# luizirber/sourmash-rust

Measured on AMD Instinct MI355X. Metric: k-mers hashed/sec (k=31, scaled=1000), higher is better.
Workload: dtype u64

## Files before the change

sourmash-rust_amd/csrc/device.cpp:

```cpp
#include "device.hpp"

#include <cstdlib>
#include <cstring>

namespace smh {

void throw_hip(hipError_t e, const char* what, const char* file, int line) {
  std::string m = std::string("HIP error ") + hipGetErrorName(e) + " (" + hipGetErrorString(e) +
                  ") in " + what + " at " + file + ":" + std::to_string(line);
  throw_internal(m);
}

namespace {
std::mutex g_pool_mu;
std::map<std::pair<int, size_t>, std::vector<void*>> g_pool;
size_t g_pool_bytes = 0;
size_t g_pool_limit = [] {
  if (const char* e = std::getenv("SOURMASH_AMD_POOL_MB")) return (size_t)std::strtoull(e, nullptr, 10) << 20;
  return (size_t)1 << 30;
}();

size_t size_class(size_t need) {
  if (need <= 4096) return 4096;
  const int lg = 63 - __builtin_clzll((unsigned long long)(need - 1));
// ... 63 lines not shown
}
size_t device_pool_bytes() {
  std::lock_guard<std::mutex> lock(g_pool_mu);
  return g_pool_bytes;
}

void DeviceBuffer::ensure(size_t need) {
  if (need <= bytes) return;
  const size_t want = need + need / 4 + 4096;
  release();
  ptr = device_pool_alloc(want, &bytes);
}
void DeviceBuffer::release() {
  if (ptr) device_pool_free(ptr, bytes, true);
  ptr = nullptr;
  bytes = 0;
}
void DeviceBuffer::release_after_sync() {
  if (ptr) device_pool_free(ptr, bytes, false);
  ptr = nullptr;
  bytes = 0;
}
DeviceBuffer::~DeviceBuffer() { release(); }

void PinnedBuffer::ensure(size_t need) {
  if (need <= bytes) return;
  size_t want = need + need / 4 + 4096;
  if (ptr) { HIP_CHECK(hipHostFree(ptr)); ptr = nullptr; bytes = 0; }
  HIP_CHECK(hipHostMalloc(&ptr, want, hipHostMallocDefault));
  bytes = want;
}
PinnedBuffer::~PinnedBuffer() { if (ptr) (void)hipHostFree(ptr); }

static int pick_device() {
  if (const char* e = std::getenv("SOURMASH_AMD_DEVICE")) return std::atoi(e);
  int cur = 0;
  if (hipGetDevice(&cur) == hipSuccess) return cur;
  return 0;
}

Device::Device() {
  int n = 0;
  hipError_t e = hipGetDeviceCount(&n);
  if (e != hipSuccess || n <= 0)
    throw_internal("no HIP device available: the sourmash MI355X library needs a GPU (" +
                   std::string(e == hipSuccess ? "device count is 0" : hipGetErrorString(e)) + ")");
  device_ = pick_device();
  if (device_ < 0 || device_ >= n) device_ = 0;
  HIP_CHECK(hipSetDevice(device_));
  hipDeviceProp_t p;
  HIP_CHECK(hipGetDeviceProperties(&p, device_));
  cus_ = p.multiProcessorCount > 0 ? p.multiProcessorCount : 256;
  HIP_CHECK(hipStreamCreateWithFlags(&stream_, hipStreamNonBlocking));
  HIP_CHECK(hipStreamCreateWithFlags(&copy_stream_, hipStreamNonBlocking));
  HIP_CHECK(hipEventCreateWithFlags(&fence_, hipEventDisableTiming));
  HIP_CHECK(hipEventCreateWithFlags(&ev_fork_, hipEventDisableTiming));
  HIP_CHECK(hipEventCreateWithFlags(&ev_join_, hipEventDisableTiming));
  HIP_CHECK(hipEventCreateWithFlags(&open_event_, hipEventDisableTiming));
}

void Device::leave_open(hipStream_t s) {
  std::lock_guard<std::recursive_mutex> lock(mu_);
  HIP_CHECK(hipEventRecord(open_event_, s));
  open_stream_ = s;
  open_ = true;
}

void Device::order_after_open(hipStream_t s) {
  std::lock_guard<std::recursive_mutex> lock(mu_);
  if (!open_) return;
  if (hipEventQuery(open_event_) == hipSuccess) { open_ = false; return; }
  if (s != open_stream_) HIP_CHECK(hipStreamWaitEvent(s, open_event_, 0));
}

hipStream_t Device::user_stream(void* given) {
  std::lock_guard<std::recursive_mutex> lock(mu_);
  if (given) { order_after_open((hipStream_t)given); return (hipStream_t)given; }
  HIP_CHECK(hipEventRecord(fence_, nullptr));
  HIP_CHECK(hipStreamWaitEvent(stream_, fence_, 0));
  order_after_open(stream_);
  return stream_;
}

Device& Device::get() {
  static Device* d = new Device();
  (void)hipSetDevice(d->device_);
  return *d;
}

bool Device::available() {
  try {
    (void)get();
    return true;
  } catch (const Error&) {
    return false;
  }
}

void Device::profile_enable(bool on) { profiling_ = on; }

void Device::prof_begin(hipStream_t s) {
  if (!profiling_) return;
  HIP_CHECK(hipEventCreate(&cur_start_));
  HIP_CHECK(hipEventRecord(cur_start_, s));
}

void Device::prof_end(const char* name, hipStream_t s) {
  if (!profiling_ || !cur_start_) return;
  hipEvent_t b;
  HIP_CHECK(hipEventCreate(&b));
  HIP_CHECK(hipEventRecord(b, s));
  pending_.push_back({name, cur_start_, b});
  cur_start_ = nullptr;
  if (pending_.size() > 4096) drain();
}

void Device::drain() {
  for (auto& p : pending_) {
    float ms = 0.f;
    if (hipEventSynchronize(p.b) == hipSuccess && hipEventElapsedTime(&ms, p.a, p.b) == hipSuccess) {
      auto& t = times_[p.name];
      t.ms += ms;
      t.launches += 1;
    }
    (void)hipEventDestroy(p.a);
    (void)hipEventDestroy(p.b);
  }
  pending_.clear();
}

void Device::count(const char* name) {
  std::lock_guard<std::recursive_mutex> lock(mu_);
  times_[name].launches += 1;
}

KernelTimes Device::prof_get(const std::string& name) {
  drain();
  auto it = times_.find(name);
  return it == times_.end() ? KernelTimes{} : it->second;
}

void Device::prof_reset() {
  drain();
  times_.clear();
}

}
```

sourmash-rust_amd/csrc/device.hpp:

```cpp
#pragma once
#include <hip/hip_runtime.h>

#include <cstddef>
#include <cstdint>
#include <map>
#include <mutex>
#include <string>
#include <vector>

#include "common.hpp"

namespace smh {

[[noreturn]] void throw_hip(hipError_t e, const char* what, const char* file, int line);

#define HIP_CHECK(expr)                                                  \
  do {                                                                   \
    hipError_t e_ = (expr);                                              \
    if (e_ != hipSuccess) ::smh::throw_hip(e_, #expr, __FILE__, __LINE__); \
  } while (0)

void* device_pool_alloc(size_t need, size_t* cap);
void device_pool_free(void* ptr, size_t cap, bool sync);
void device_pool_trim();
void device_pool_set_limit(size_t bytes);
size_t device_pool_bytes();

struct PoolBlock {
  void* ptr = nullptr;
  size_t cap = 0;
  bool synced = false;
  explicit PoolBlock(size_t bytes) { ptr = device_pool_alloc(bytes ? bytes : 1, &cap); }
  PoolBlock(const PoolBlock&) = delete; PoolBlock& operator=(const PoolBlock&) = delete;
  ~PoolBlock() { device_pool_free(ptr, cap, !synced); }
  template <class T> T* as() const { return reinterpret_cast<T*>(ptr); }
};

struct DeviceBuffer {
  void* ptr = nullptr;
  size_t bytes = 0;
  void ensure(size_t need);
  void release();
  void release_after_sync();
  template <class T> T* as() const { return reinterpret_cast<T*>(ptr); }
  DeviceBuffer() = default;
  DeviceBuffer(const DeviceBuffer&) = delete;
  DeviceBuffer& operator=(const DeviceBuffer&) = delete;
  ~DeviceBuffer();
};

struct PinnedBuffer {
  void* ptr = nullptr;
  size_t bytes = 0;
  void ensure(size_t need);
  template <class T> T* as() const { return reinterpret_cast<T*>(ptr); }
  PinnedBuffer() = default;
  PinnedBuffer(const PinnedBuffer&) = delete;
  PinnedBuffer& operator=(const PinnedBuffer&) = delete;
  ~PinnedBuffer();
};

struct KernelTimes {
  double ms = 0.0;
  uint64_t launches = 0;
};

class Device {
 public:
  static Device& get();
  static bool available();

  int id() const { return device_; }
  int cu_count() const { return cus_; }
  hipStream_t stream() { order_after_open(stream_); return stream_; }
  hipStream_t copy_stream() const { return copy_stream_; }
  hipEvent_t fork_event() const { return ev_fork_; }
  hipEvent_t join_event() const { return ev_join_; }
  void leave_open(hipStream_t s);
  void order_after_open(hipStream_t s);
  hipStream_t user_stream(void* given);
  std::recursive_mutex& mutex() { return mu_; }

  DeviceBuffer scratch;
  DeviceBuffer tile_rec;

  void profile_enable(bool on);
  bool profiling() const { return profiling_; }
  void prof_begin(hipStream_t s);
  void prof_end(const char* name, hipStream_t s);
  void count(const char* name);
  KernelTimes prof_get(const std::string& name);
  void prof_reset();

 private:
  Device();
  int device_ = 0;
  int cus_ = 256;
  hipStream_t stream_ = nullptr;
  hipStream_t copy_stream_ = nullptr;
  hipEvent_t fence_ = nullptr;
  hipEvent_t ev_fork_ = nullptr, ev_join_ = nullptr;
  hipEvent_t open_event_ = nullptr;
  hipStream_t open_stream_ = nullptr;
  bool open_ = false;
  std::recursive_mutex mu_;
  bool profiling_ = false;
  struct Pending { std::string name; hipEvent_t a, b; };
  std::vector<Pending> pending_;
  hipEvent_t cur_start_ = nullptr;
  std::map<std::string, KernelTimes> times_;
  void drain();
};

}
```

sourmash-rust_amd/csrc/sketch_kernels.hip:

```cpp
#include <hip/hip_runtime.h>
#include <stdint.h>

#include <cstdio>
#include <cstdlib>
#include <type_traits>

#include "device.hpp"
#include "kernels.hpp"

namespace smh {
namespace {

constexpr uint64_t kC1 = 0x87c37b91114253d5ULL;
constexpr uint64_t kC2 = 0x4cf5ad432745937fULL;

__device__ __forceinline__ uint64_t rotl64(uint64_t x, int r) { return (x << r) | (x >> (64 - r)); }
__device__ __forceinline__ uint64_t fmix64(uint64_t k) {
  k ^= k >> 33;
  k *= 0xff51afd7ed558ccdULL;
  k ^= k >> 33;
  k *= 0xc4ceb9fe1a85ec53ULL;
  k ^= k >> 33;
  return k;
}
// ... 185 lines not shown
  k = w2_mul(k, 0xff51afd7ed558ccdULL);
  k.lo ^= k.hi >> 1;
  k = w2_mul(k, 0xc4ceb9fe1a85ec53ULL);
  return k;
}
__device__ __forceinline__ uint32_t open_thr(uint64_t thr) {
  const uint32_t hi = (uint32_t)(thr >> 32);
  return hi == 0xffffffffu ? hi : hi + 1u;
}
__device__ __forceinline__ bool open_may_pass(W2 a, W2 b, uint32_t thr_hi1) { return a.hi + b.hi + 1u <= thr_hi1; }
__device__ __forceinline__ uint64_t open_finish(W2 a, W2 b) {
  a.lo ^= a.hi >> 1; b.lo ^= b.hi >> 1;
  return ((((uint64_t)a.hi << 32) | a.lo) + (((uint64_t)b.hi << 32) | b.lo));
}
__device__ __forceinline__ W2 w2_add_keep(W2 a, W2 b) {
  uint64_t r;
  asm("v_lshl_add_u64 %0, %1, 0, %2" : "=v"(r) : "v"(((uint64_t)a.hi << 32) | a.lo), "v"(((uint64_t)b.hi << 32) | b.lo));
  return w2_split(r);
}
constexpr uint64_t kFmixC2 = 0xc4ceb9fe1a85ec53ULL;
__device__ __forceinline__ W2 w2_fmix_pre(W2 k) {
  k.lo ^= k.hi >> 1;
  k = w2_mul(k, 0xff51afd7ed558ccdULL);
  k.lo ^= k.hi >> 1;
  return k;
}
__device__ __forceinline__ uint32_t open_hi_sum1(W2 ka, W2 kb) {
  const uint32_t cl = (uint32_t)kFmixC2, ch = (uint32_t)(kFmixC2 >> 32);
  uint64_t s0, s1, s2, s3, cy;
  asm("v_mad_u64_u32 %0, %1, %2, %3, 1" : "=v"(s0), "=s"(cy) : "v"(ka.hi), "s"(cl));
  asm("v_mad_u64_u32 %0, %1, %2, %3, %4" : "=v"(s1), "=s"(cy) : "v"(ka.lo), "s"(ch), "v"(s0));
  asm("v_mad_u64_u32 %0, %1, %2, %3, %4" : "=v"(s2), "=s"(cy) : "v"(kb.hi), "s"(cl), "v"(s1));
  asm("v_mad_u64_u32 %0, %1, %2, %3, %4" : "=v"(s3), "=s"(cy) : "v"(kb.lo), "s"(ch), "v"(s2));
  return (uint32_t)s3 + __umulhi(ka.lo, cl) + __umulhi(kb.lo, cl);
}
__device__ __forceinline__ uint64_t open_full(W2 ka, W2 kb) { return open_finish(w2_mul(ka, kFmixC2), w2_mul(kb, kFmixC2)); }
__device__ __forceinline__ W2 mix_k1_fold(uint32_t S, W2 T) {
  const uint32_t cl = (uint32_t)kC2, ch = (uint32_t)(kC2 >> 32), s1 = S >> 1;
  uint64_t p, cy;
  asm("v_mad_u64_u32 %0, %1, %2, %3, %4" : "=v"(p), "=s"(cy) : "v"(s1), "s"(cl), "v"(((uint64_t)T.hi << 32) | T.lo));
  uint32_t hi, top;
  asm("v_add_u32 %0, %1, %2" : "=v"(hi) : "v"((uint32_t)(p >> 32)), "v"(s1 * ch));
  asm("v_lshl_add_u32 %0, %1, 31, %2" : "=v"(top) : "v"(S), "v"(hi));
  return {(uint32_t)p, top};
}
template <bool CROSS>
__device__ __forceinline__ W2 mix_k2_fold(uint32_t S, W2 T, uint32_t Bp) {
  const uint32_t cl = (uint32_t)kC1x2, ch = (uint32_t)(kC1x2 >> 32);
  uint64_t p, cy;
  asm("v_mad_u64_u32 %0, %1, %2, %3, %4" : "=v"(p), "=s"(cy) : "v"(S), "s"(cl), "v"(((uint64_t)T.hi << 32) | T.lo));
  uint32_t hi;
  asm("v_add_u32 %0, %1, %2" : "=v"(hi) : "v"((uint32_t)(p >> 32)), "v"(CROSS ? Bp : S * ch));
  return {(uint32_t)p, hi};
}
template <bool FOLD, bool CROSS>
__device__ __forceinline__ W2 mix_word(int w, W2 M, uint32_t S, uint32_t P) {
  if (FOLD) return (w & 1) ? mix_k2_fold<CROSS>(S, M, P) : mix_k1_fold(S, M);
  return (w & 1) ? w2_mul(w2_rotl(M, 33), kC1) : w2_mul(w2_rotl(M, 31), kC2);
}
template <int L, bool FOLD, bool CROSS>
__device__ __forceinline__ void murmur_kmer_pre(const W2 (&M)[2 * L], const uint32_t (&S)[2 * L], const uint32_t (&P)[2 * L], int K, uint64_t seed, W2 seedv,
                                                W2& a, W2& b) {
  W2 h1 = seedv, h2 = seedv;
  const int nblocks = K >> 4, tail = K & 15;
#pragma unroll
  for (int blk = 0; blk < L; blk++) {
    const int w1 = 2 * blk, w2 = 2 * blk + 1;
    if (blk < nblocks) {
      h1 = w2_xor(h1, mix_word<FOLD, CROSS>(w1, M[w1], S[w1], P[w1]));
      if (blk == 0) h1 = w2_mul5_add(w2_rotl(h1, 27), seed * 5 + 0x52dce729u);
      else h1 = w2_mul5_add(w2_add(w2_rotl(h1, 27), h2), 0x52dce729u);
      h2 = w2_xor(h2, mix_word<FOLD, CROSS>(w2, M[w2], S[w2], P[w2]));
      h2 = w2_mul5_add(w2_add_keep(w2_rotl(h2, 31), h1), 0x38495ab5u);
    } else if (blk == nblocks) {
      if (tail > 8) h2 = w2_xor(h2, mix_word<FOLD, CROSS>(w2, M[w2], S[w2], P[w2]));
      if (tail > 0) h1 = w2_xor(h1, mix_word<FOLD, CROSS>(w1, M[w1], S[w1], P[w1]));
    }
  }
  h1.lo ^= (uint32_t)K; h2.lo ^= (uint32_t)K;
  w2_cross_add(h1, h2);
  a = w2_fmix_pre(h1); b = w2_fmix_pre(h2);
}

template <int KT, int THREADS, int HB, int L, bool PR = false, bool PK = false, int MINW = (PK ? 8 : 4)>
__global__ __launch_bounds__(THREADS, MINW) void k_dna_rolling(SeqBatch b, HashParams hp, CandSink sink,
                                                                     int logR, uint32_t stage_cap) {
  constexpr bool FOLD = PK && L == 2;
  constexpr bool CROSS = FOLD && !PR;
  __shared__ __attribute__((aligned(16))) uint32_t lut[CROSS ? kLutDwordsCross : (FOLD ? kLutDwordsFold : kLutDwords)];
  extern __shared__ __attribute__((aligned(16))) uint32_t smem[];
  uint32_t* st_ctl = smem;
  uint64_t* st_hash = reinterpret_cast<uint64_t*>(st_ctl + 4);
  uint64_t* st_pos = st_hash + stage_cap;
  uint32_t* tile = reinterpret_cast<uint32_t*>(st_pos + (sink.pos ? stage_cap : 0));
  const Stage stage{st_ctl, st_hash, st_pos, stage_cap};

  const int K = KT ? KT : (int)hp.ksize;
  const int tid = threadIdx.x;
  const uint32_t R = 1u << logR;
  const uint64_t TILE = (uint64_t)THREADS << logR;
  uint32_t MASK[L];
#pragma unroll
  for (int i = 0; i < L; i++) {
    const int bits = 2 * K - 32 * i;
    MASK[i] = bits >= 32 ? 0xffffffffu : (bits <= 0 ? 0u : ((1u << bits) - 1u));
  }
  const int top_limb = (2 * K - 2) >> 5, top_sh = (2 * K - 2) & 31;
  const bool multi = b.starts != nullptr;

  const int g_last = (K - 1) >> 2, nb_last = K - 4 * g_last;
  const uint64_t c_last = ((g_last >> 1) & 1) ? kC2 : kC1;
  uint64_t* ptab = reinterpret_cast<uint64_t*>(lut);
  for (int e = tid; e < kLutEntries; e += THREADS) {
    const uint32_t ent = (uint32_t)e;
    const uint32_t idx = ent & 255u;
    const int nb = ent < 512 ? 4 : (ent < 576 ? nb_last : 0);
    uint32_t v = 0;
    for (int j = 0; j < nb; j++) v |= ((0x54474341u >> (8 * ((idx >> (2 * j)) & 3))) & 0xffu) << (8 * j);
    const uint64_t c = ent < 256 ? kC1 : (ent < 512 ? kC2 : c_last);
    const uint64_t prod = (uint64_t)v * c;
    if (FOLD) {
      const uint64_t mm = (uint32_t)prod;
      const uint32_t ahi = (uint32_t)(prod >> 32), ch = (uint32_t)(kC1x2 >> 32);
      const uint64_t t = c == kC1 ? (mm << 31) * kC2
                                  : ((mm >> 31) | ((mm & 0x7fffffffu) << 33)) * kC1 + (CROSS ? (uint64_t)(ahi * ch) << 32 : 0ull);
      reinterpret_cast<uint4*>(lut)[e] = make_uint4((uint32_t)t, (uint32_t)(t >> 32), ahi, 0u);
      const uint32_t B = (uint32_t)prod;
      const uint32_t he = ent < 256 ? ent : ent - 256u;
      if (!CROSS) lut[4 * kLutEntries + e] = B;
      else {
        if (ent < 256 || ent >= 512) lut[kLutFoldB4 + he] = B;
        if (ent >= 256) reinterpret_cast<uint2*>(lut + kLutFoldB8)[he] = make_uint2(B, B * ch);
      }
    } else {
      ptab[e] = prod;
      lut[2 * kLutEntries + e] = (uint32_t)prod;
    }
  }
  uint32_t gbase[4 * L];
#pragma unroll
  for (int g = 0; g < 4 * L; g++) {
    const int nb = K - 4 * g;
    uint32_t ent0 = 576u;
    if (nb >= 4) ent0 = ((g >> 1) & 1) ? 256u : 0u;
    else if (nb > 0) ent0 = 512u;
    constexpr uint32_t esz = FOLD ? 16u : 8u;
    gbase[g] = (g & 1) ? esz * kLutEntries + ent0 * 4u : ent0 * esz;
    if (CROSS && (g & 1)) {
      const uint32_t he = nb >= 4 ? 0u : (nb > 0 ? 256u : 320u);
      gbase[g] = (g & 2) ? 4u * kLutFoldB8 + he * 8u : 4u * kLutFoldB4 + he * 4u;
    }
  }
  if (tid == 0) st_ctl[0] = 0;

  const uint64_t span = hp.range_hi - hp.range_lo;
  const uint64_t ntiles = (span + TILE - 1) / TILE;
  const uintptr_t gend = ((uintptr_t)(b.seq + b.len) + 15) & ~(uintptr_t)15;
  const uint32_t nsteps = (R + (uint32_t)K - 1 + 3) & ~3u;
  const uint32_t warm_end = K > 4 ? ((uint32_t)(K - 1) & ~3u) : 0u;

  for (uint64_t tix = blockIdx.x; tix < ntiles; tix += gridDim.x) {
    const uint64_t T0 = hp.range_lo + tix * TILE;
    const uint64_t thr = hp.thr;
    const uint32_t thr_hi1 = open_thr(hp.thr);
    W2 seedv{(uint32_t)hp.seed, (uint32_t)(hp.seed >> 32)};
    asm volatile("" : "+v"(seedv.lo), "+v"(seedv.hi));
    uint64_t lthr = hp.thr;

    const uintptr_t g0 = (uintptr_t)(b.seq + T0);
    const uintptr_t ga = g0 & ~(uintptr_t)15;
    const uint32_t m = (uint32_t)(g0 - ga);
    const uint32_t nchunks = (m + (uint32_t)TILE + 16 * L + 8 + 15 + (PK ? 32u : 0u)) >> 4;
    const uint32_t nchunks_cap = (15u + (uint32_t)TILE + 16 * L + 8 + 15 + 32u) >> 4;
    __syncthreads();
    uint32_t* dirty = tile + (nchunks_cap + (nchunks_cap >> (logR - 4)) + 2);
    if (PK) {
      for (uint32_t c = tid; c < (nchunks >> 3) + 3; c += THREADS) dirty[c] = 0;
      if (tid == 0) st_ctl[1] = 0;
      __syncthreads();
    }
    const uint64_t cin64 = gend > ga ? (uint64_t)(gend - ga) >> 4 : 0ull;
    const uint32_t cin = cin64 < nchunks ? (uint32_t)cin64 : nchunks;
    uint32_t kActg;
    asm("s_mov_b32 %0, 0x47544341" : "=s"(kActg));
    for (uint32_t c = tid; c < nchunks; c += THREADS) {
      uint4 v = make_uint4(0, 0, 0, 0);
      if (c < cin) v = *reinterpret_cast<const uint4*>(ga + ((uintptr_t)c << 4));
      if (PK) {
        const uint32_t w4[4] = {v.x, v.y, v.z, v.w};
        uint32_t xany = 0, gray = 0;
#pragma unroll
        for (int q = 0; q < 4; q++) {
          const uint32_t u4 = w4[q] & 0xDFDFDFDFu;
          const uint32_t g4 = (u4 >> 1) & 0x03030303u;
          xany |= u4 ^ __builtin_amdgcn_perm(0u, kActg, g4);
          gray |= __builtin_amdgcn_udot4(g4, 0x40100401u, 0u, false) << (8 * q);
        }
        tile[c + (c >> (logR - 4))] = gray ^ ((gray >> 1) & 0x55555555u);
        if (xany) {
          const volatile uint32_t* src = reinterpret_cast<const volatile uint32_t*>(ga + ((uintptr_t)c << 4));
          uint32_t bad = 0;
#pragma unroll
          for (int q = 0; q < 4; q++) {
            const uint32_t u4 = (c < cin ? src[q] : 0u) & 0xDFDFDFDFu;
            bad |= u4 != __builtin_amdgcn_perm(0u, kActg, (u4 >> 1) & 0x03030303u) ? 1u << q : 0u;
          }
          atomicOr(&dirty[c >> 3], bad << (4u * (c & 7u)));
          st_ctl[1] = 1;
        }
      } else {
        uint32_t x = c << 4;
        uint32_t o = (x >> 2) + (x >> logR);
        tile[o] = v.x; tile[o + 1] = v.y; tile[o + 2] = v.z; tile[o + 3] = v.w;
      }
    }
    __syncthreads();

    const uint64_t p0 = T0 + ((uint64_t)tid << logR);
    if (p0 < hp.range_hi) {
    const uint32_t nk = (hp.range_hi - p0) < R ? (uint32_t)(hp.range_hi - p0) : R;
    const uint32_t hi_ok = nk + (uint32_t)K - 1;

    uint32_t rec = 0;
    uint64_t cur_end = b.vend0;
    if (multi) {
      rec = find_record_in_tile(b, 0, tix, p0, &cur_end);
      if (PR) lthr = hp.thr_rec[rec];
    }
    uint32_t lim = 0;
    if (cur_end > p0) lim = (cur_end - p0) > 0xfffffffeull ? 0xffffffffu : (uint32_t)(cur_end - p0);
    uint32_t vstart = 0;
    uint32_t g_lo = 0, g_span = 0;
    uint64_t dmask = 0;
    if (PK && st_ctl[1]) {
      const uint32_t b0 = (m + ((uint32_t)tid << logR)) >> 2;
      const uint32_t* dw = reinterpret_cast<const uint32_t*>(tile) + (nchunks_cap + (nchunks_cap >> (logR - 4)) + 2);
      const uint32_t i = b0 >> 5, sft = b0 & 31u;
      const uint64_t lo64 = ((uint64_t)dw[i + 1] << 32) | dw[i];
      const uint32_t d2 = dw[i + 2];
      dmask = (lo64 >> sft) | (sft ? ((uint64_t)d2 << (64 - sft)) : 0ull);
      if (m & 3u) dmask |= (dmask >> 1) | ((uint64_t)((d2 >> sft) & 1u) << 63);
    }
    constexpr bool kEdgeFree = KT > 0 && (KT - 1) % HB == 0;
    auto set_clean_window = [&](bool warm, uint32_t from_i) {
      const bool whole = warm || (kEdgeFree && vstart == 0 && nk == R);
      uint32_t lim2 = whole ? lim : (lim < hi_ok ? lim : hi_ok);
      if (PK) {
        const uint32_t g = from_i >> 2;
        const uint64_t rem = g < 64 ? (dmask >> g) : 0ull;
        if (rem) lim2 = min(lim2, (g + (uint32_t)__builtin_ctzll(rem)) * 4u);
      }
      g_lo = whole ? vstart : vstart + (uint32_t)K - 1;
      g_span = lim2 >= g_lo + 4 ? lim2 - 3 - g_lo : 0u;
    };

    const uint32_t xu = m & ~3u;
    uint32_t ta = xu + ((uint32_t)tid << logR);
    ta = ta + ((ta >> logR) << 2);
    const uint32_t sh = m & 3u;
    uint32_t cur = PK ? 0u : tile[ta >> 2];
    uint32_t cq = (m >> 4) + ((uint32_t)tid << (logR - 4));
    const uint32_t sh2 = (m & 15u) * 2u;
    uint32_t pcur = PK ? tile[cq + (cq >> (logR - 4))] : 0u, w = 0, wc = 0;
    uint32_t cf[L], fle[L];
#pragma unroll
    for (int i = 0; i < L; i++) { cf[i] = 0; fle[i] = 0; }
    constexpr bool kRoll31 = PK && L == 2 && KT == 31;
    constexpr bool kMinF64 = PK && L == 2 && KT > 0 && KT <= 31;
    uint32_t fa0 = 0, fa1 = 0, cs0 = 0, cs1 = 0, wr = 0;

    auto group = [&](uint32_t i0, auto hashing) {
      constexpr bool kHash = decltype(hashing)::value;
      uint32_t code4 = 0, ccode4 = 0, diff4 = 0;
      if (PK) {
        if ((i0 & 12u) == 0) {
          cq += 1;
          const uint32_t pnxt = tile[cq + (cq >> (logR - 4))];
          w = __builtin_amdgcn_alignbit(pnxt, pcur, sh2);
          pcur = pnxt;
          wc = ~w;
          if (kRoll31) {
            fa1 |= w << 30;
            const uint32_t r = __builtin_bitreverse32(w);
            wr = ~(((r >> 1) & 0x55555555u) | ((r << 1) & 0xaaaaaaaau));
          }
        }
      } else {
        const uint32_t xn = xu + i0 + 4;
        ta += (xn & (R - 1)) == 0 ? 8u : 4u;
        const uint32_t nxt = tile[ta >> 2];
        const uint32_t d = __builtin_amdgcn_alignbyte(nxt, cur, sh);
        cur = nxt;
        const uint32_t u4 = d & 0xDFDFDFDFu;
        const uint32_t c2 = (u4 >> 1) & 0x03030303u;
        code4 = c2 ^ ((c2 >> 1) & 0x01010101u);
        const uint32_t exp4 = __builtin_amdgcn_perm(0u, 0x54474341u, code4);
        diff4 = u4 ^ exp4;
        ccode4 = code4 ^ 0x03030303u;
      }
// ... 84 lines not shown
              for (int li = 0; li < L; li++) X[q][li] = fwd ? fle[li] : cf[li];
            }
          }
        }
        if (kHash && i0 + g0b + HB >= (uint32_t)K && i0 + g0b < R + (uint32_t)K - 1) {
          W2 ha[HB], hb[HB];
#pragma unroll
          for (int q = 0; q < HB; q++) {
            W2 M[2 * L];
            uint32_t S[2 * L], P[2 * L];
#pragma unroll
            for (int wi = 0; wi < 2 * L; wi++) { M[wi] = W2{0u, 0u}; S[wi] = 0u; P[wi] = 0u; }
#pragma unroll
            for (int g = 0; g < 4 * L; g++) {
              if (KT == 0 || 4 * g < K) {
                const uint32_t xw = X[q][g >> 2];
                uint32_t off;
                if ((g & 3) == 0 && FOLD) asm("v_lshlrev_b32_sdwa %0, 4, %1 dst_sel:DWORD dst_unused:UNUSED_PAD src0_sel:DWORD src1_sel:BYTE_0" : "=v"(off) : "v"(xw));
                else if ((g & 3) == 0) asm("v_lshlrev_b32_sdwa %0, 3, %1 dst_sel:DWORD dst_unused:UNUSED_PAD src0_sel:DWORD src1_sel:BYTE_0" : "=v"(off) : "v"(xw));
                else if ((g & 3) == 1) asm("v_lshlrev_b32_sdwa %0, 2, %1 dst_sel:DWORD dst_unused:UNUSED_PAD src0_sel:DWORD src1_sel:BYTE_1" : "=v"(off) : "v"(xw));
                else if ((g & 3) == 2 && FOLD) asm("v_lshlrev_b32_sdwa %0, 4, %1 dst_sel:DWORD dst_unused:UNUSED_PAD src0_sel:DWORD src1_sel:BYTE_2" : "=v"(off) : "v"(xw));
                else if ((g & 3) == 2) asm("v_lshlrev_b32_sdwa %0, 3, %1 dst_sel:DWORD dst_unused:UNUSED_PAD src0_sel:DWORD src1_sel:BYTE_2" : "=v"(off) : "v"(xw));
                else if ((g & 3) == 3 && CROSS) asm("v_lshlrev_b32_sdwa %0, 3, %1 dst_sel:DWORD dst_unused:UNUSED_PAD src0_sel:DWORD src1_sel:BYTE_3" : "=v"(off) : "v"(xw));
                else asm("v_lshlrev_b32_sdwa %0, 2, %1 dst_sel:DWORD dst_unused:UNUSED_PAD src0_sel:DWORD src1_sel:BYTE_3" : "=v"(off) : "v"(xw));
                const char* at = reinterpret_cast<const char*>(lut) + gbase[g] + off;
                if ((g & 1) == 0 && FOLD) {
                  typedef uint32_t u32x4 __attribute__((ext_vector_type(4)));
                  u32x4 e = *reinterpret_cast<const u32x4*>(at);
                  asm("" : "+v"(e));
                  M[g >> 1] = W2{e.x, e.y};
                  S[g >> 1] = e.z;
                } else if ((g & 1) == 0) {
                  const uint2 e = *reinterpret_cast<const uint2*>(at);
                  M[g >> 1] = W2{e.x, e.y};
                } else if (CROSS && (g & 2)) {
                  const uint2 e = *reinterpret_cast<const uint2*>(at);
                  S[g >> 1] += e.x;
                  P[g >> 1] = e.y;
                } else if (FOLD) {
                  S[g >> 1] += *reinterpret_cast<const uint32_t*>(at);
                } else {
                  M[g >> 1].hi += *reinterpret_cast<const uint32_t*>(at);
                }
              }
            }
            murmur_kmer_pre<L, FOLD, CROSS>(M, S, P, K, hp.seed, seedv, ha[q], hb[q]);
          }
#pragma unroll
          for (int q = 0; q < HB; q++)
            if (open_hi_sum1(ha[q], hb[q]) <= (PR ? open_thr(tq[g0b + q]) : thr_hi1)) {
              uint32_t om = okmask;
              asm volatile("" : "+v"(om));
              const uint64_t h = open_full(ha[q], hb[q]);
              if (h <= (PR ? tq[g0b + q] : thr) && ((om >> (g0b + q)) & 1u))
                stage_emit(stage, sink, h, hp.pos_base + p0 + (i0 + g0b + q + 1 - (uint32_t)K));
            }
        }
      }
      if (PK) { w >>= 8; wc >>= 8; }
      if (kRoll31) wr <<= 8;
    };

    set_clean_window(true, 0);
    if (kRoll31 && !PR && g_span > 24u) {
      const uint32_t d1 = tile[cq + 1 + ((cq + 1) >> (logR - 4))], d2 = tile[cq + 2 + ((cq + 2) >> (logR - 4))];
      const uint32_t q0 = __builtin_amdgcn_alignbit(d1, pcur, sh2), q1 = __builtin_amdgcn_alignbit(d2, d1, sh2);
      cq += 2; pcur = d2;
      fa0 = q0 << 6;
      fa1 = __builtin_amdgcn_alignbit(q1, q0, 26);
      const uint32_t r0 = __builtin_bitreverse32(q0), r1 = __builtin_bitreverse32(q1);
      const uint32_t c0 = ~(((r0 >> 1) & 0x55555555u) | ((r0 << 1) & 0xaaaaaaaau));
      const uint32_t c1 = ~(((r1 >> 1) & 0x55555555u) | ((r1 << 1) & 0xaaaaaaaau));
      cs0 = __builtin_amdgcn_alignbit(c0, c1, 8);
      cs1 = c0 >> 8;
      w = q1 >> 24; wc = ~q1 >> 24; wr = c1 << 24;
    } else {
      for (uint32_t i0 = 0; i0 < warm_end; i0 += 4) group(i0, std::false_type{});
    }
    set_clean_window(false, warm_end);
    for (uint32_t i0 = warm_end; i0 < nsteps; i0 += 4) group(i0, std::true_type{});
    }

    stage_flush(stage, sink, tid, THREADS);
  }
}

__global__ __launch_bounds__(256) void k_dna_generic(SeqBatch b, HashParams hp, CandSink sink) {
  const uint64_t K = hp.ksize;
  const uint64_t stride = (uint64_t)gridDim.x * blockDim.x;
  for (uint64_t p = hp.range_lo + (uint64_t)blockIdx.x * blockDim.x + threadIdx.x; p < hp.range_hi;
       p += stride) {
    uint64_t end = b.vend0, thr = hp.thr;
    if (b.starts) {
      uint32_t r = find_record(b.starts, b.nrec, p);
      end = b.vends ? b.vends[r] : b.starts[r + 1];
      if (hp.thr_rec) thr = hp.thr_rec[r];
    }
    if (p + K > end || p + K < p) continue;
    const uint8_t* s = b.seq + p;
    bool ok = true, decided = false, fwd = true;
    for (uint64_t i = 0; i < K; i++) {
      uint32_t f = upper(s[i]);
      if (!(f == 'A' || f == 'C' || f == 'G' || f == 'T')) { ok = false; break; }
      if (!decided) {
        uint32_t t = upper(s[K - 1 - i]);
        uint32_t rc = t == 'A' ? 'T' : t == 'T' ? 'A' : t == 'C' ? 'G' : t == 'G' ? 'C' : t;
        if (f != rc) { fwd = f < rc; decided = true; }
      }
    }
    if (!ok) continue;
    Mm3Stream st(hp.seed);
    for (uint64_t i = 0; i < K; i++) {
      uint32_t c;
      if (fwd) c = upper(s[i]);
      else {
        uint32_t t = upper(s[K - 1 - i]);
        c = t == 'A' ? 'T' : t == 'T' ? 'A' : t == 'C' ? 'G' : 'C';
      }
      st.push(c);
    }
    uint64_t h = st.finish();
    if (h <= thr) emit(sink, h, hp.pos_base + p);
  }
}

__global__ __launch_bounds__(256) void k_first_invalid(SeqBatch b, uint64_t* __restrict__ vends) {
  const uintptr_t p0 = (uintptr_t)b.seq, pa = p0 & ~(uintptr_t)15;
  const uint64_t head = p0 - pa;
  const uint64_t nch = (head + b.len + 15) >> 4;
  const uint64_t stride = (uint64_t)gridDim.x * blockDim.x;
  for (uint64_t c = (uint64_t)blockIdx.x * blockDim.x + threadIdx.x; c < nch; c += stride) {
    const uint4 v = *reinterpret_cast<const uint4*>(pa + (c << 4));
    const uint32_t w[4] = {v.x, v.y, v.z, v.w};
#pragma unroll
    for (int k = 0; k < 4; k++) {
      const uint32_t u4 = w[k] & 0xDFDFDFDFu;
      const uint32_t c2 = (u4 >> 1) & 0x03030303u;
      const uint32_t code4 = c2 ^ ((c2 >> 1) & 0x01010101u);
      const uint32_t diff4 = u4 ^ __builtin_amdgcn_perm(0u, 0x54474341u, code4);
      if (diff4 == 0) continue;
      for (int j = 0; j < 4; j++) {
        if (((diff4 >> (8 * j)) & 0xffu) == 0) continue;
        const uint64_t at = (c << 4) + 4 * k + j;
        if (at < head || at - head >= b.len) continue;
        const uint64_t q = at - head;
        const uint32_t r = b.starts ? find_record(b.starts, b.nrec, q) : 0;
        atomicMin((unsigned long long*)&vends[r], (unsigned long long)q);
      }
    }
  }
}
__global__ __launch_bounds__(256) void k_first_bad_record(const uint64_t* __restrict__ starts, const uint64_t* __restrict__ vends,
                                                          uint32_t nrec, uint32_t ksize, unsigned long long* __restrict__ out) {
  unsigned long long best = ~0ull;
  for (uint64_t r = (uint64_t)blockIdx.x * blockDim.x + threadIdx.x; r < nrec; r += (uint64_t)gridDim.x * blockDim.x) {
    const uint64_t st = starts[r], en = starts[r + 1];
    if (vends[r] < en && en - st >= ksize && r < best) best = r;
  }
  for (int off = 32; off; off >>= 1) {
    const unsigned long long o = __shfl_down(best, off);
    best = o < best ? o : best;
  }
  if ((threadIdx.x & 63) == 0 && best != ~0ull) atomicMin(out, best);
}

constexpr uint32_t kDropped = 0xFFu;
// ... 765 lines not shown
    if (p + win > end || p + win < p) continue;
    Mm3Stream st(hp.seed);
    for (uint32_t i = 0; i < win; i++) st.push(lut[b.seq[p + i]]);
    const uint64_t h = st.finish();
    if (h <= hp.thr) emit(sink, h, hp.pos_base + p);
  }
}

__global__ __launch_bounds__(256) void k_hash_segments(const uint8_t* __restrict__ bytes,
                                                       const uint64_t* __restrict__ off, uint32_t nseg,
                                                       uint64_t seed, uint64_t* __restrict__ out) {
  uint32_t i = blockIdx.x * blockDim.x + threadIdx.x;
  if (i >= nseg) return;
  Mm3Stream st(seed);
  for (uint64_t q = off[i]; q < off[i + 1]; q++) st.push(bytes[q]);
  out[i] = st.finish();
}

__global__ __launch_bounds__(256) void k_filter_hashes(const uint64_t* __restrict__ hashes, HashParams hp, CandSink sink) {
  const uint64_t stride = (uint64_t)gridDim.x * blockDim.x;
  const uint64_t thr = hp.thr;
  for (uint64_t i = hp.range_lo + (uint64_t)blockIdx.x * blockDim.x + threadIdx.x; i < hp.range_hi; i += stride) {
    const uint64_t h = hashes[i];
    if (h <= thr) emit(sink, h, hp.pos_base + i);
  }
}

__device__ __forceinline__ uint64_t splitmix64(uint64_t seed, uint64_t index) {
  uint64_t z = seed + (index + 1) * 0x9E3779B97F4A7C15ULL;
  z = (z ^ (z >> 30)) * 0xBF58476D1CE4E5B9ULL;
  z = (z ^ (z >> 27)) * 0x94D049BB133111EBULL;
  return z ^ (z >> 31);
}

__global__ __launch_bounds__(256) void k_synth_dna(uint8_t* __restrict__ out, uint64_t start, uint64_t len,
                                                   uint64_t seed, uint64_t n_every) {
  const uint64_t nwords = (len + 31) / 32;
  const uint64_t stride = (uint64_t)gridDim.x * blockDim.x;
  for (uint64_t w = (uint64_t)blockIdx.x * blockDim.x + threadIdx.x; w < nwords; w += stride) {
    uint64_t bits = splitmix64(seed, (start >> 5) + w);
    uint64_t p = start + 32 * w;
    uint64_t nrem = n_every ? p % n_every : 0;
    uint64_t o = 32 * w;
    for (int j = 0; j < 32 && o + j < len; j++) {
      uint32_t c = (0x54474341u >> (8 * ((bits >> (2 * j)) & 3))) & 0xffu;
      if (n_every) {
        if (nrem == n_every - 1) c = 'N';
        nrem = nrem + 1 == n_every ? 0 : nrem + 1;
      }
      out[o + j] = (uint8_t)c;
    }
  }
}

inline int grid_for(uint64_t items, int per_block, int cap) {
  uint64_t g = (items + per_block - 1) / per_block;
  if (g < 1) g = 1;
  if (g > (uint64_t)cap) g = cap;
  return (int)g;
}

}


struct DnaCfg { int threads, logR, hb; bool packed = true; };
static DnaCfg dna_cfg() {
  static DnaCfg cfg = [] {
    DnaCfg c{512, 7, 2};
#ifdef SMH_EXPERIMENTS
    if (const char* e = std::getenv("SOURMASH_AMD_DNA_PK")) c.packed = std::atoi(e) != 0;
#endif
#ifdef SMH_EXPERIMENTS
    if (const char* e = std::getenv("SOURMASH_AMD_DNA_CFG")) {
      int t = 0, r = 0, h = 0;
      if (sscanf(e, "%d,%d,%d", &t, &r, &h) == 3 && (t == 256 || t == 512) && r >= 5 && r <= 7 &&
          (h == 1 || h == 2 || h == 4)) c = DnaCfg{t, r, h, false};
    }
#endif
    return c;
  }();
  return cfg;
}

template <int KT, int L>
static void launch_rolling(const SeqBatch& b, const HashParams& p, const CandSink& sink, int grid, size_t lds,
                           int logR, uint32_t stage_cap, const DnaCfg& c, hipStream_t s) {
#define SMH_LAUNCH(T, H) hipLaunchKernelGGL((k_dna_rolling<KT, T, H, L>), dim3(grid), dim3(T), lds, s, b, p, sink, logR, stage_cap)
  if (p.thr_rec) {
    if (c.packed) hipLaunchKernelGGL((k_dna_rolling<KT, 512, 2, L, true, true>), dim3(grid), dim3(512), lds, s, b, p, sink, logR, stage_cap);
    else hipLaunchKernelGGL((k_dna_rolling<KT, 512, 2, L, true>), dim3(grid), dim3(512), lds, s, b, p, sink, logR, stage_cap);
    return;
  }
  if (c.packed) {
#ifdef SMH_EXPERIMENTS
    if (const char* e = std::getenv("SOURMASH_AMD_DNA_PKV")) {
      int mw = 0, hb = 0;
      if (sscanf(e, "%d,%d", &mw, &hb) == 2) {
#define SMH_PKV(M_, H_) if (mw == M_ && hb == H_) { hipLaunchKernelGGL((k_dna_rolling<KT, 512, H_, L, false, true, M_>), dim3(grid), dim3(512), lds, s, b, p, sink, logR, stage_cap); return; }
        SMH_PKV(8, 1) SMH_PKV(7, 1) SMH_PKV(6, 1) SMH_PKV(5, 1) SMH_PKV(4, 1) SMH_PKV(8, 2) SMH_PKV(6, 2) SMH_PKV(5, 2) SMH_PKV(4, 2) SMH_PKV(8, 4) SMH_PKV(6, 4)
#undef SMH_PKV
      }
    }
#endif
    hipLaunchKernelGGL((k_dna_rolling<KT, 512, 1, L, false, true, 6>), dim3(grid), dim3(512), lds, s, b, p, sink, logR, stage_cap);
    return;
  }
#ifdef SMH_EXPERIMENTS
  if (c.threads == 512) { if (c.hb == 4) SMH_LAUNCH(512, 4); else if (c.hb == 2) SMH_LAUNCH(512, 2); else SMH_LAUNCH(512, 1); }
  else { if (c.hb == 4) SMH_LAUNCH(256, 4); else if (c.hb == 2) SMH_LAUNCH(256, 2); else SMH_LAUNCH(256, 1); }
#else
  SMH_LAUNCH(512, 2);
#endif
#undef SMH_LAUNCH
}

static SeqBatch with_tile_records(const SeqBatch& b, uint32_t min_len, uint64_t base, uint64_t tile, uint64_t ntiles, Device& dev,
                                  hipStream_t s) {
  SeqBatch r = b;
  if (!b.starts || b.nrec < 2) return r;
  dev.tile_rec.ensure((size_t)ntiles * sizeof(TileRec));
  hipLaunchKernelGGL(k_tile_records, dim3((unsigned)((ntiles + 255) / 256)), dim3(256), 0, s, b.starts, b.vends, b.nrec, min_len, base,
                     tile, ntiles, dev.tile_rec.as<TileRec>());
  r.tile_rec = dev.tile_rec.as<TileRec>();
  return r;
}

void launch_dna_hash(const SeqBatch& b_in, const HashParams& p, const CandSink& sink, Device& dev,
                     hipStream_t s, bool force_generic) {
  if (p.range_hi <= p.range_lo) return;
  const uint64_t span = p.range_hi - p.range_lo;
  if (p.ksize >= 1 && p.ksize <= 128 && !force_generic) {
    DnaCfg c = dna_cfg();
    if (p.thr_rec) { c.threads = 512; c.logR = 7; c.hb = 2; }
    int logR = c.logR;
    while (logR > 5 && (span >> logR) < (uint64_t)dev.cu_count() * c.threads * 2) logR--;
    const uint64_t tile = (uint64_t)c.threads << logR;
    const uint64_t ntiles = (span + tile - 1) / tile;
    const SeqBatch b = with_tile_records(b_in, 0, p.range_lo, tile, ntiles, dev, s);
    dev.prof_begin(s);
    int grid = (int)(ntiles < (uint64_t)dev.cu_count() * 8 ? ntiles : (uint64_t)dev.cu_count() * 8);
    const int limbs = p.ksize <= 32 ? 2 : (p.ksize <= 64 ? 4 : 8);
    const uint32_t x_bytes = (uint32_t)tile + 16 * limbs + 96;
    const uint64_t thr = p.thr;
    long double expect = (long double)tile * (((long double)thr + 1.0L) / 18446744073709551616.0L);
    uint32_t stage_cap = expect * 2.0L + 64.0L > 2048.0L ? 2048u : (uint32_t)(expect * 2.0L + 64.0L);
    if (stage_cap < 128) stage_cap = 128;
    size_t lds = 16 + (size_t)stage_cap * 8 * (sink.pos ? 2 : 1) + x_bytes +
                 4 * ((x_bytes >> logR) + 2);
    if (c.packed) {
      const uint32_t ncap = (15u + (uint32_t)tile + 16u * (uint32_t)limbs + 8u + 15u + 32u) >> 4;
      lds = 16 + (size_t)stage_cap * 8 * (sink.pos ? 2 : 1) + 4 * (size_t)(ncap + (ncap >> (logR - 4)) + 2) + 4 * (size_t)((ncap >> 3) + 8);
    }
    if (p.ksize == 31) launch_rolling<31, 2>(b, p, sink, grid, lds, logR, stage_cap, c, s);
    else if (p.ksize == 21) launch_rolling<21, 2>(b, p, sink, grid, lds, logR, stage_cap, c, s);
    else if (p.ksize == 51) launch_rolling<51, 4>(b, p, sink, grid, lds, logR, stage_cap, c, s);
    else if (p.ksize <= 32) launch_rolling<0, 2>(b, p, sink, grid, lds, logR, stage_cap, c, s);
    else if (p.ksize <= 64) launch_rolling<0, 4>(b, p, sink, grid, lds, logR, stage_cap, c, s);
    else launch_rolling<0, 8>(b, p, sink, grid, lds, logR, stage_cap, c, s);
    HIP_CHECK(hipGetLastError());
    dev.prof_end("dna_rolling", s);
  } else {
    dev.prof_begin(s);
    hipLaunchKernelGGL(k_dna_generic, dim3(grid_for(span, 256, dev.cu_count() * 16)), dim3(256), 0, s,
                       b_in, p, sink);
    HIP_CHECK(hipGetLastError());
    dev.prof_end("dna_generic", s);
  }
}

__global__ __launch_bounds__(256) void k_record_stats(const uint64_t* __restrict__ starts, uint32_t nrec, uint32_t ksize,
                                                      unsigned long long* __restrict__ out) {
  unsigned long long nlong = 0, total = 0;
  for (uint64_t r = (uint64_t)blockIdx.x * blockDim.x + threadIdx.x; r < nrec; r += (uint64_t)gridDim.x * blockDim.x) {
    const uint64_t len = starts[r + 1] - starts[r];
    if (len >= ksize) {
      nlong++;
      if (len >= 2) total += 2 * (len - 2);
      else for (uint32_t f = 0; f < 3; f++) total += len >= f ? 2 * ((len - f) / 3) : 0;
    }
  }
  for (int off = 32; off; off >>= 1) { nlong += __shfl_down(nlong, off); total += __shfl_down(total, off); }
  if ((threadIdx.x & 63) == 0 && (nlong | total)) { atomicAdd(&out[0], nlong); atomicAdd(&out[1], total); }
}
void launch_record_stats(const uint64_t* starts, uint32_t nrec, uint32_t ksize, uint64_t* out2, hipStream_t s) {
  HIP_CHECK(hipMemsetAsync(out2, 0, 16, s));
  hipLaunchKernelGGL(k_record_stats, dim3(grid_for(nrec, 256, 2048)), dim3(256), 0, s, starts, nrec, ksize,
                     reinterpret_cast<unsigned long long*>(out2));
  HIP_CHECK(hipGetLastError());
}

void launch_first_bad_record(const uint64_t* starts, const uint64_t* vends, uint32_t nrec, uint32_t ksize, uint64_t* out, hipStream_t s) {
  HIP_CHECK(hipMemsetAsync(out, 0xff, 8, s));
  hipLaunchKernelGGL(k_first_bad_record, dim3(grid_for(nrec, 256, 2048)), dim3(256), 0, s, starts, vends, nrec, ksize,
                     reinterpret_cast<unsigned long long*>(out));
  HIP_CHECK(hipGetLastError());
}

void launch_first_invalid(const SeqBatch& b, uint64_t* vends_out, hipStream_t s) {
  if (b.len == 0) return;
  hipLaunchKernelGGL(k_first_invalid, dim3(grid_for(b.len + 32, 256 * 16, 8192)), dim3(256), 0, s, b,
                     vends_out);
  HIP_CHECK(hipGetLastError());
}

void launch_translate(const SeqBatch& b, const uint64_t* seg_off, uint32_t nseg, uint64_t total, uint32_t ksize, uint32_t alphabet,
                      uint8_t* residues, uint32_t* bad_utf8, hipStream_t s) {
  if (total == 0) return;
  hipLaunchKernelGGL(k_translate, dim3(grid_for(b.len, kTrTile, 16384)), dim3(kTrThreads), 0, s, b, seg_off, nseg, ksize, alphabet,
                     residues, bad_utf8);
  HIP_CHECK(hipGetLastError());
}

bool launch_protein_fused(const SeqBatch& b_in, const uint64_t* seg_offsets, uint32_t win, const HashParams& p,
                          const CandSink& sink, uint32_t* high_flag, Device& dev, hipStream_t s) {
  if (b_in.len == 0) return true;
  if (!(win == 7 || win == 9 || win == 10)) return false;
  int logR = SMH_PF_LOGR;
  while (logR > 5 && (b_in.len >> logR) < (uint64_t)dev.cu_count() * 512 * 2) logR--;
  const uint64_t tile = 512ull << logR;
  const uint64_t ntiles = (b_in.len + tile - 1) / tile;
  const int grid = (int)(ntiles < (uint64_t)dev.cu_count() * 8 ? ntiles : (uint64_t)dev.cu_count() * 8);
  const uint32_t x_bytes = (uint32_t)tile + 3 * win + 12 + 96;
  long double expect = 2.0L * (long double)tile * (((long double)p.thr + 1.0L) / 18446744073709551616.0L);
  uint32_t stage_cap = expect * 2.0L + 64.0L > 2048.0L ? 2048u : (uint32_t)(expect * 2.0L + 64.0L);
  if (stage_cap < 128) stage_cap = 128;
  const size_t lds = 16 + (size_t)stage_cap * 8 * (sink.pos ? 2 : 1) + x_bytes + 4 * ((x_bytes >> logR) + 2);
  const SeqBatch b = with_tile_records(b_in, p.ksize, 0, tile, ntiles, dev, s);
  dev.scratch.ensure(16 + (size_t)kSplicedCap * 8);
  uint32_t* slow_count = dev.scratch.as<uint32_t>();
  uint64_t* slow_list = reinterpret_cast<uint64_t*>(dev.scratch.as<char>() + 16);
  HIP_CHECK(hipMemsetAsync(slow_count, 0, 4, s));
#define SMH_PF(W_) hipLaunchKernelGGL((k_protein_fused<W_, 512>), dim3(grid), dim3(512), lds, s, b, p, sink, logR, stage_cap, high_flag, \
                                      slow_list, slow_count)
  if (win == 7) SMH_PF(7); else if (win == 9) SMH_PF(9); else SMH_PF(10);
#undef SMH_PF
  hipLaunchKernelGGL(k_spliced_windows, dim3(64), dim3(256), 0, s, b, p, sink, win, slow_list, slow_count);
  if (sink.pos)
    hipLaunchKernelGGL(k_protein_positions, dim3(dev.cu_count() * 4), dim3(256), 0, s, sink.pos, sink.count, sink.capacity, b.starts,
                       b.nrec, b.len, seg_offsets, 3 * win, p.pos_base);
  HIP_CHECK(hipGetLastError());
  return true;
// ... 73 lines not shown
```

Baseline: 420.1 billion.

## Schedule DNA rolling-hash tiles dynamically with an atomic counter and occupancy-sized grid

The grid for the rolling DNA hash kernel is now sized to the number of workgroups that fit on the device at once, using the occupancy query. Before, it was a fixed cu_count*8. Workgroups then claim further tiles through a global atomic counter instead of a fixed grid stride. The counter is zeroed per launch by a memset on the stream. The aim is to cut load imbalance and tail effects across compute units. In exchange it adds one atomic per tile, one extra memset per launch, and a slightly larger LDS control header.

New measurement: 449.8 billion, median of 6. 7.1% higher.

```diff
diff --git a/sourmash-rust_amd/csrc/device.cpp b/sourmash-rust_amd/csrc/device.cpp
--- a/sourmash-rust_amd/csrc/device.cpp
+++ b/sourmash-rust_amd/csrc/device.cpp
@@ -169,6 +169,15 @@
   return stream_;
 }
 
+uint32_t* Device::tile_counter(hipStream_t s) {
+  std::lock_guard<std::recursive_mutex> lock(mu_);
+  tile_counters_.ensure(kTileCounters * sizeof(uint32_t));
+  uint32_t* w = tile_counters_.as<uint32_t>() + tile_counter_next_;
+  tile_counter_next_ = (tile_counter_next_ + 1) % kTileCounters;
+  HIP_CHECK(hipMemsetAsync(w, 0, sizeof(uint32_t), s));
+  return w;
+}
+
 Device& Device::get() {
   static Device* d = new Device();
   (void)hipSetDevice(d->device_);
diff --git a/sourmash-rust_amd/csrc/device.hpp b/sourmash-rust_amd/csrc/device.hpp
--- a/sourmash-rust_amd/csrc/device.hpp
+++ b/sourmash-rust_amd/csrc/device.hpp
@@ -83,6 +83,8 @@
 
   DeviceBuffer scratch;
   DeviceBuffer tile_rec;
+  static constexpr uint32_t kTileCounters = 64;
+  uint32_t* tile_counter(hipStream_t s);
 
   void profile_enable(bool on);
   bool profiling() const { return profiling_; }
@@ -104,6 +106,8 @@
   hipStream_t open_stream_ = nullptr;
   bool open_ = false;
   std::recursive_mutex mu_;
+  DeviceBuffer tile_counters_;
+  uint32_t tile_counter_next_ = 0;
   bool profiling_ = false;
   struct Pending { std::string name; hipEvent_t a, b; };
   std::vector<Pending> pending_;
diff --git a/sourmash-rust_amd/csrc/sketch_kernels.hip b/sourmash-rust_amd/csrc/sketch_kernels.hip
--- a/sourmash-rust_amd/csrc/sketch_kernels.hip
+++ b/sourmash-rust_amd/csrc/sketch_kernels.hip
@@ -291,15 +291,16 @@
   a = w2_fmix_pre(h1); b = w2_fmix_pre(h2);
 }
 
+constexpr int kDnaCtlDwords = 8;
 template <int KT, int THREADS, int HB, int L, bool PR = false, bool PK = false, int MINW = (PK ? 8 : 4)>
 __global__ __launch_bounds__(THREADS, MINW) void k_dna_rolling(SeqBatch b, HashParams hp, CandSink sink,
-                                                                     int logR, uint32_t stage_cap) {
+                                                                     int logR, uint32_t stage_cap, uint32_t* tile_ctr) {
   constexpr bool FOLD = PK && L == 2;
   constexpr bool CROSS = FOLD && !PR;
   __shared__ __attribute__((aligned(16))) uint32_t lut[CROSS ? kLutDwordsCross : (FOLD ? kLutDwordsFold : kLutDwords)];
   extern __shared__ __attribute__((aligned(16))) uint32_t smem[];
   uint32_t* st_ctl = smem;
-  uint64_t* st_hash = reinterpret_cast<uint64_t*>(st_ctl + 4);
+  uint64_t* st_hash = reinterpret_cast<uint64_t*>(st_ctl + kDnaCtlDwords);
   uint64_t* st_pos = st_hash + stage_cap;
   uint32_t* tile = reinterpret_cast<uint32_t*>(st_pos + (sink.pos ? stage_cap : 0));
   const Stage stage{st_ctl, st_hash, st_pos, stage_cap};
@@ -368,7 +369,7 @@
   const uint32_t nsteps = (R + (uint32_t)K - 1 + 3) & ~3u;
   const uint32_t warm_end = K > 4 ? ((uint32_t)(K - 1) & ~3u) : 0u;
 
-  for (uint64_t tix = blockIdx.x; tix < ntiles; tix += gridDim.x) {
+  for (uint64_t tix = blockIdx.x; tix < ntiles;) {
     const uint64_t T0 = hp.range_lo + tix * TILE;
     const uint64_t thr = hp.thr;
     const uint32_t thr_hi1 = open_thr(hp.thr);
@@ -424,6 +425,7 @@
       }
     }
     __syncthreads();
+    if (!PR && tile_ctr && tid == 0) st_ctl[4] = atomicAdd(tile_ctr, 1u);
 
     const uint64_t p0 = T0 + ((uint64_t)tid << logR);
     if (p0 < hp.range_hi) {
@@ -674,6 +676,8 @@
     }
 
     stage_flush(stage, sink, tid, THREADS);
+    if (!PR && tile_ctr) tix = (uint64_t)gridDim.x + (uint32_t)__builtin_amdgcn_readfirstlane((int)st_ctl[4]);
+    else tix += gridDim.x;
   }
 }
 
@@ -1605,13 +1609,48 @@
   return cfg;
 }
 
+template <class Kernel>
+static uint64_t resident_workgroups(Kernel kernel, int threads, size_t lds, Device& dev) {
+  static std::mutex mu;
+  static std::map<std::pair<const void*, size_t>, int> cache;
+  std::lock_guard<std::mutex> lock(mu);
+  const auto key = std::make_pair(reinterpret_cast<const void*>(kernel), lds);
+  auto it = cache.find(key);
+  if (it == cache.end()) {
+    int per_cu = 0;
+    HIP_CHECK(hipOccupancyMaxActiveBlocksPerMultiprocessor(&per_cu, kernel, threads, lds));
+    if (per_cu < 1) throw_internal("a sketch kernel does not fit a compute unit (occupancy query)");
+    it = cache.emplace(key, per_cu).first;
+  }
+  return (uint64_t)it->second * (uint64_t)dev.cu_count();
+}
+
+template <class Kernel>
+static void launch_rolling_tiles(Kernel kernel, int threads, bool per_record, const SeqBatch& b, const HashParams& p, const CandSink& sink,
+                                 uint64_t ntiles, size_t lds, int logR, uint32_t stage_cap, Device& dev, hipStream_t s) {
+  uint64_t grid = per_record ? (uint64_t)dev.cu_count() * 8 : resident_workgroups(kernel, threads, lds, dev);
+  bool dynamic = !per_record && ntiles > grid && ntiles < (1ull << 31);
+#ifdef SMH_EXPERIMENTS
+  if (const char* e = per_record ? nullptr : std::getenv("SOURMASH_AMD_DNA_GRID")) {
+    if (std::atoi(e) > 0) grid = (uint64_t)dev.cu_count() * (uint64_t)std::atoi(e);
+    dynamic = false;
+  }
+#endif
+  if (grid > ntiles) grid = ntiles;
+  uint32_t* ctr = dynamic ? dev.tile_counter(s) : nullptr;
+  dev.count(dynamic ? "dna_tiles_dynamic" : "dna_tiles_static");
+  dev.prof_begin(s);
+  hipLaunchKernelGGL(kernel, dim3((unsigned)grid), dim3(threads), lds, s, b, p, sink, logR, stage_cap, ctr);
+}
+
 template <int KT, int L>
-static void launch_rolling(const SeqBatch& b, const HashParams& p, const CandSink& sink, int grid, size_t lds,
-                           int logR, uint32_t stage_cap, const DnaCfg& c, hipStream_t s) {
-#define SMH_LAUNCH(T, H) hipLaunchKernelGGL((k_dna_rolling<KT, T, H, L>), dim3(grid), dim3(T), lds, s, b, p, sink, logR, stage_cap)
+static void launch_rolling(const SeqBatch& b, const HashParams& p, const CandSink& sink, uint64_t ntiles, size_t lds,
+                           int logR, uint32_t stage_cap, const DnaCfg& c, Device& dev, hipStream_t s) {
+#define SMH_LAUNCH_K(T, ...) launch_rolling_tiles(k_dna_rolling<KT, T, __VA_ARGS__>, T, p.thr_rec != nullptr, b, p, sink, ntiles, lds, logR, stage_cap, dev, s)
+#define SMH_LAUNCH(T, H) SMH_LAUNCH_K(T, H, L)
   if (p.thr_rec) {
-    if (c.packed) hipLaunchKernelGGL((k_dna_rolling<KT, 512, 2, L, true, true>), dim3(grid), dim3(512), lds, s, b, p, sink, logR, stage_cap);
-    else hipLaunchKernelGGL((k_dna_rolling<KT, 512, 2, L, true>), dim3(grid), dim3(512), lds, s, b, p, sink, logR, stage_cap);
+    if (c.packed) SMH_LAUNCH_K(512, 2, L, true, true);
+    else SMH_LAUNCH_K(512, 2, L, true);
     return;
   }
   if (c.packed) {
@@ -1619,13 +1658,13 @@
     if (const char* e = std::getenv("SOURMASH_AMD_DNA_PKV")) {
       int mw = 0, hb = 0;
       if (sscanf(e, "%d,%d", &mw, &hb) == 2) {
-#define SMH_PKV(M_, H_) if (mw == M_ && hb == H_) { hipLaunchKernelGGL((k_dna_rolling<KT, 512, H_, L, false, true, M_>), dim3(grid), dim3(512), lds, s, b, p, sink, logR, stage_cap); return; }
+#define SMH_PKV(M_, H_) if (mw == M_ && hb == H_) { SMH_LAUNCH_K(512, H_, L, false, true, M_); return; }
         SMH_PKV(8, 1) SMH_PKV(7, 1) SMH_PKV(6, 1) SMH_PKV(5, 1) SMH_PKV(4, 1) SMH_PKV(8, 2) SMH_PKV(6, 2) SMH_PKV(5, 2) SMH_PKV(4, 2) SMH_PKV(8, 4) SMH_PKV(6, 4)
 #undef SMH_PKV
       }
     }
 #endif
-    hipLaunchKernelGGL((k_dna_rolling<KT, 512, 1, L, false, true, 6>), dim3(grid), dim3(512), lds, s, b, p, sink, logR, stage_cap);
+    SMH_LAUNCH_K(512, 1, L, false, true, 6);
     return;
   }
 #ifdef SMH_EXPERIMENTS
@@ -1635,6 +1674,7 @@
   SMH_LAUNCH(512, 2);
 #endif
 #undef SMH_LAUNCH
+#undef SMH_LAUNCH_K
 }
 
 static SeqBatch with_tile_records(const SeqBatch& b, uint32_t min_len, uint64_t base, uint64_t tile, uint64_t ntiles, Device& dev,
@@ -1660,26 +1700,24 @@
     const uint64_t tile = (uint64_t)c.threads << logR;
     const uint64_t ntiles = (span + tile - 1) / tile;
     const SeqBatch b = with_tile_records(b_in, 0, p.range_lo, tile, ntiles, dev, s);
-    dev.prof_begin(s);
-    int grid = (int)(ntiles < (uint64_t)dev.cu_count() * 8 ? ntiles : (uint64_t)dev.cu_count() * 8);
     const int limbs = p.ksize <= 32 ? 2 : (p.ksize <= 64 ? 4 : 8);
     const uint32_t x_bytes = (uint32_t)tile + 16 * limbs + 96;
     const uint64_t thr = p.thr;
     long double expect = (long double)tile * (((long double)thr + 1.0L) / 18446744073709551616.0L);
     uint32_t stage_cap = expect * 2.0L + 64.0L > 2048.0L ? 2048u : (uint32_t)(expect * 2.0L + 64.0L);
     if (stage_cap < 128) stage_cap = 128;
-    size_t lds = 16 + (size_t)stage_cap * 8 * (sink.pos ? 2 : 1) + x_bytes +
+    size_t lds = 4 * kDnaCtlDwords + (size_t)stage_cap * 8 * (sink.pos ? 2 : 1) + x_bytes +
                  4 * ((x_bytes >> logR) + 2);
     if (c.packed) {
       const uint32_t ncap = (15u + (uint32_t)tile + 16u * (uint32_t)limbs + 8u + 15u + 32u) >> 4;
-      lds = 16 + (size_t)stage_cap * 8 * (sink.pos ? 2 : 1) + 4 * (size_t)(ncap + (ncap >> (logR - 4)) + 2) + 4 * (size_t)((ncap >> 3) + 8);
-    }
-    if (p.ksize == 31) launch_rolling<31, 2>(b, p, sink, grid, lds, logR, stage_cap, c, s);
-    else if (p.ksize == 21) launch_rolling<21, 2>(b, p, sink, grid, lds, logR, stage_cap, c, s);
-    else if (p.ksize == 51) launch_rolling<51, 4>(b, p, sink, grid, lds, logR, stage_cap, c, s);
-    else if (p.ksize <= 32) launch_rolling<0, 2>(b, p, sink, grid, lds, logR, stage_cap, c, s);
-    else if (p.ksize <= 64) launch_rolling<0, 4>(b, p, sink, grid, lds, logR, stage_cap, c, s);
-    else launch_rolling<0, 8>(b, p, sink, grid, lds, logR, stage_cap, c, s);
+      lds = 4 * kDnaCtlDwords + (size_t)stage_cap * 8 * (sink.pos ? 2 : 1) + 4 * (size_t)(ncap + (ncap >> (logR - 4)) + 2) + 4 * (size_t)((ncap >> 3) + 8);
+    }
+    if (p.ksize == 31) launch_rolling<31, 2>(b, p, sink, ntiles, lds, logR, stage_cap, c, dev, s);
+    else if (p.ksize == 21) launch_rolling<21, 2>(b, p, sink, ntiles, lds, logR, stage_cap, c, dev, s);
+    else if (p.ksize == 51) launch_rolling<51, 4>(b, p, sink, ntiles, lds, logR, stage_cap, c, dev, s);
+    else if (p.ksize <= 32) launch_rolling<0, 2>(b, p, sink, ntiles, lds, logR, stage_cap, c, dev, s);
+    else if (p.ksize <= 64) launch_rolling<0, 4>(b, p, sink, ntiles, lds, logR, stage_cap, c, dev, s);
+    else launch_rolling<0, 8>(b, p, sink, ntiles, lds, logR, stage_cap, c, dev, s);
     HIP_CHECK(hipGetLastError());
     dev.prof_end("dna_rolling", s);
   } else {
```
